# lpiccinelli-eth/UniDepth

Hardware: AMD Instinct MI355X
Metric: images/sec (whole node) + p50 latency, ViT-L/14 518x518 bs=8 (higher is better)
Workload: dtype f16; 1 GPU; UniDepthV2 vitl14 infer(), 518x518, bs=8 per GPU, all 7 outputs on device; value = 2 independent infer() calls in flight per GPU (HIP streams); value_one_call / p50_latency_ms = one call at a time; global_batch=8, parallelism=dp1, inflight=2

## Files before the change

unidepth_amd/csrc/gemm.hip:

```cpp
#include "ud_common.h"

#ifdef UD_TRACE
__device__ unsigned long long* ud_trace_ptr = nullptr;
#define UD_STAMP(slot)                                                                           \
  do {                                                                                           \
    if (ud_trace_ptr && threadIdx.x == 0 && trace_tile < 8)                                      \
      ud_trace_ptr[((size_t)blockIdx.x * 8 + trace_tile) * 8 + (slot)] = wall_clock64();         \
  } while (0)
#else
#define UD_STAMP(slot)
#endif

namespace {

constexpr int UD_LNC_TILES = 2;
constexpr int UD_LNC_PLANE = UD_LNC_TILES * 256;

template <int BN_, int WM_, int WN_>
struct Cfg {
  static constexpr int BM = 128, BN = BN_, BK = 64, WM = WM_, WN = WN_;
  static constexpr int NWM = BM / WM, NWN = BN / WN;
  static constexpr int TM = WM / 16, TN = WN / 16;
  static constexpr int A_BYTES = BM * BK * 2;
  static constexpr int B_BYTES = BN * BK * 2;
// ... 1397 lines not shown
    }
  }
  hipLaunchKernelGGL((gemm256_kernel<MH, EPI, AMODE, false, LNC, GRP>), dim3(tiles < 256 ? tiles : 256), dim3(512), lds, s, d);
  UD_CHECK_LAUNCH("ud_gemm_f16 (large tile) launch");
  return UD_OK;
}

inline int bal_cpc(const UdGemm& d) {
  const int tiles_n = (d.N + 255) >> 8;
  if (tiles_n > 128 || (d.N & 255)) return 0;
  const int cpc = 256 / tiles_n;
  const int U = (d.M + 63) >> 6;
  return (U / cpc >= 2) ? cpc : 0;
}
inline double bal_time(const UdGemm& d) {
  const int cpc = bal_cpc(d);
  if (!cpc) return 1e30;
  const int U = (d.M + 63) >> 6;
  const int un = (U + cpc - 1) / cpc;
  const int k = (un + 3) >> 2;
  return 8.0 + (un * (30.0 / 4.0) + (k - 1) * 2.5) * ((double)d.K / 1024.0);
}

template <int EPI, bool LNC = false, int AMODE = UD_A_DENSE>
int launch256bal(const UdGemm& d, hipStream_t s) {
  const int tiles_n = (d.N + 255) >> 8;
  const int cpc = bal_cpc(d);
  const int lds = 2 * BigCfg<4>::STAGE + (LNC ? LNC_LDS : 0);
  static bool attr_set[UD_MAX_DEVICES];
  if (!ud_attr_once(attr_set)) {
    if (hipFuncSetAttribute((const void*)gemm256_kernel<4, EPI, AMODE, true, LNC>, hipFuncAttributeMaxDynamicSharedMemorySize, lds) != hipSuccess) {
      ud_set_error("ud_gemm_f16: cannot reserve the LDS ring of the large-tile kernel");
      return UD_ERR_LAUNCH;
    }
  }
  hipLaunchKernelGGL((gemm256_kernel<4, EPI, AMODE, true, LNC>), dim3(cpc * tiles_n), dim3(512), lds, s, d);
  UD_CHECK_LAUNCH("ud_gemm_f16 (large tile, row-balanced) launch");
  return UD_OK;
}

inline int pick_tiles(const UdGemm& d) {
  if (d.amode == UD_A_CONV3_REFLECT || d.groups > 1 || d.M < 1024 || d.N < 192 || (d.K & 63)) return 0;
  if (d.amode == UD_A_CONV3_ZERO && d.epi != UD_EPI_F16 && d.epi != UD_EPI_F32) return 0;
  {
    const double a_bytes = d.amode == UD_A_DENSE ? 2.0 * d.M * d.lda : 2.0 * ((double)(d.M / d.rows_img) + 1.0) * (double)d.img_stride;
    if (a_bytes >= 2147483648.0 || 2.0 * d.N * d.ldw >= 2147483648.0) return 0;
  }
  if (d.epi == UD_EPI_QKV && (d.vsplit & 255)) return 0;
  if (d.tile_hint == 1 || (d.tile_hint >= 5 && d.tile_hint != 8 && d.tile_hint != 9 && d.tile_hint != 10 && (d.tile_hint < 11 || d.tile_hint > 14))) return 0;
  if (d.tile_hint >= 11 && d.tile_hint <= 14) return 3;
  if (d.tile_hint == 2) return 4;
  if (d.tile_hint == 10) return big_split_ok(d) ? 10 : 0;
  if (d.tile_hint == 3 || d.tile_hint == 9) return 3;
  const bool bal_ok = (d.amode == UD_A_DENSE || (d.amode == UD_A_CONV3_ZERO && d.epi != UD_EPI_QKV)) &&
                      (d.epi == UD_EPI_F16 || d.epi == UD_EPI_F32 || d.epi == UD_EPI_QKV) && bal_cpc(d) > 0;
  if (d.tile_hint == 8 && bal_ok) return 8;
  const double kk = (double)d.K / 1024.0;
  const double tn = (double)((d.N + 255) / 256);
  const double t256 = 8.0 + ceil(tn * ((d.M + 255) / 256) / 256.0) * 30.0 * kk;
  const double t192 = 8.0 + ceil(tn * ((d.M + 191) / 192) / 256.0) * 23.5 * kk;
  const double tbal = (bal_ok && ((d.M + 63) / 64 + bal_cpc(d) - 1) / bal_cpc(d) > 4) ? bal_time(d) : 1e30;
  const double small_tiles = (double)((d.N + 127) / 128) * ((d.M + 127) / 128);
  const double t_small = 6.0 + ceil(small_tiles / 256.0) * 0.5 * 21.5 * kk;
  double t_big = t256 <= t192 ? t256 : t192;
  int which = t256 <= t192 ? 4 : 3;
  if (tbal < 0.985 * t_big) { t_big = tbal; which = 8; }
  if (big_split_ok(d)) {
    const double tsplit = 8.0 + 0.5 * 23.5 * kk + 6.0;
    if (tsplit < t_big && tsplit < 0.93 * t_small) return 10;
  }
  if (t_big >= 0.93 * t_small) return 0;
  return which;
}

inline int big_tiles_per_wg(const UdGemm& d, int which) {
  if (which == 8) {
    const int cpc = bal_cpc(d);
    const int U = (d.M + 63) >> 6;
    return (((U + cpc - 1) / cpc) + 3) >> 2;
  }
  if (which == 10) return 1;
  const int bm = which == 3 ? 192 : 256;
  const int tiles = ((d.N + 255) >> 8) * ((d.M + bm - 1) / bm);
  return (tiles + 255) / 256;
}

template <int EPI, int AMODE = UD_A_DENSE>
int launch_big(const UdGemm& d, hipStream_t s, int which) {
  if constexpr (AMODE == UD_A_DENSE && (EPI == UD_EPI_F16 || EPI == UD_EPI_QKV)) {
    if (d.row_stats_in) {
      if (which == 8) return launch256bal<EPI, true>(d, s);
      return which == 3 ? launch256<3, EPI, AMODE, true>(d, s) : launch256<4, EPI, AMODE, true>(d, s);
    }
  }
  if constexpr (AMODE == UD_A_DENSE && (EPI == UD_EPI_F16 || EPI == UD_EPI_F32 || EPI == UD_EPI_QKV)) {
    if (which == 8 && !d.row_stats_final) return launch256bal<EPI>(d, s);
  }
  if constexpr (AMODE == UD_A_CONV3_ZERO && (EPI == UD_EPI_F16 || EPI == UD_EPI_F32)) {
    if (which == 8 && !d.row_stats_final) return launch256bal<EPI, false, UD_A_CONV3_ZERO>(d, s);
  }
  if constexpr (EPI == UD_EPI_F16 || EPI == UD_EPI_F32) {
    if (which == 10) return launch256sk<EPI, AMODE>(d, s);
  }
  if (which == 8 || which == 10) which = 3;
  return which == 3 ? launch256<3, EPI, AMODE>(d, s) : launch256<4, EPI, AMODE>(d, s);
}

constexpr int HALO_BYTES = 41 * 1024;

template <int NT, int EPI, bool REFLECT, bool UPS = false>
__global__ __launch_bounds__(256) void conv_tile_kernel(const UdGemm p) {
  extern __shared__ __attribute__((aligned(16))) char smem[];
  char* halo = smem;
  char* wbuf = smem + HALO_BYTES;
  constexpr int WB = NT * 16 * 128;
  const int tid = threadIdx.x;
  const int lane = tid & 63;
  const int wv = __builtin_amdgcn_readfirstlane(tid >> 6);
  const int tiles_x = (p.Wimg + 15) >> 4;
  const int tx = blockIdx.x % tiles_x, ty = blockIdx.x / tiles_x;
  const int x0 = tx << 4, y0 = ty << 4;
  const int b = blockIdx.y, g = blockIdx.z;
  const half_t* in = (const half_t*)p.A + (long long)g * p.gA + (long long)b * p.img_stride + p.coff;
  const half_t* W = (const half_t*)p.W + (long long)g * p.gW;
  const float* bias = p.bias + (long long)g * p.gBias;
  const float ups_sy = UPS && p.Himg > 1 ? (float)(p.Hsrc - 1) / (float)(p.Himg - 1) : 0.f;
  const float ups_sx = UPS && p.Wimg > 1 ? (float)(p.Wsrc - 1) / (float)(p.Wimg - 1) : 0.f;

  f32x4 acc[4][NT];
#pragma unroll
  for (int i = 0; i < 4; ++i)
#pragma unroll
    for (int j = 0; j < NT; ++j) acc[i][j] = (f32x4){0.f, 0.f, 0.f, 0.f};

  auto halo_coord = [&](int i, int& hp, int& cpos, int& iy, int& ix, bool& ok) {
    const int idx = i * 64 + lane;
    hp = idx >> 3;
    cpos = idx & 7;
    const int hy = hp / 18, hx = hp - hy * 18;
    iy = y0 - 1 + hy;
    ix = x0 - 1 + hx;
    ok = hp < 324;
    if constexpr (REFLECT) {
      iy = iy < 0 ? -iy : (iy >= p.Himg ? 2 * p.Himg - 2 - iy : iy);
      ix = ix < 0 ? -ix : (ix >= p.Wimg ? 2 * p.Wimg - 2 - ix : ix);
      ok = ok && iy >= 0 && ix >= 0;
    } else {
      ok = ok && (unsigned)iy < (unsigned)p.Himg && (unsigned)ix < (unsigned)p.Wimg;
    }
  };
  auto issue_halo = [&](int cc) {
    if constexpr (UPS) {
      const int ylo = y0 == 0 ? 0 : y0 - 1, yhi = y0 + 16 < p.Himg ? y0 + 16 : p.Himg - 1;
      const int xlo = x0 == 0 ? 0 : x0 - 1, xhi = x0 + 16 < p.Wimg ? x0 + 16 : p.Wimg - 1;
      const int syA = (int)(ups_sy * (float)ylo), sxA = (int)(ups_sx * (float)xlo);
      int syB = (int)(ups_sy * (float)yhi) + 1, sxB = (int)(ups_sx * (float)xhi) + 1;
      syB = syB < p.Hsrc ? syB : p.Hsrc - 1;
      sxB = sxB < p.Wsrc ? sxB : p.Wsrc - 1;
      const int PR = syB - syA + 1, PC = sxB - sxA + 1;
      char* patch = wbuf + 2 * WB;
      const int npiece = (PR * PC * 8 + 63) >> 6;
      for (int i = wv; i < npiece; i += 4) {
        const int idx = i * 64 + lane;
        int pp = idx >> 3;
        pp = pp < PR * PC ? pp : PR * PC - 1;
        const int pr = pp / PC, pc = pp - pr * PC;
        ud_glds16(in + ((long long)(syA + pr) * p.Wsrc + sxA + pc) * p.cstride + cc * 64 + ((idx & 7) << 3), patch + i * 1024);
      }
      asm volatile("s_waitcnt vmcnt(0)" ::: "memory");
      __syncthreads();
#pragma unroll
      for (int j = 0; j < 11; ++j) {
        const int i = wv + 4 * j;
        if (i < 41) {
          int hp, cpos, iy, ix;
          bool ok;
          halo_coord(i, hp, cpos, iy, ix, ok);
          ok = ok && iy >= ylo && iy <= yhi && ix >= xlo && ix <= xhi;
          half8 o8;
#pragma unroll
          for (int e = 0; e < 8; ++e) o8[e] = (half_t)0.f;
          if (ok) {
            const float fy = ups_sy * (float)iy, fx = ups_sx * (float)ix;
            const int sy0 = (int)fy, sx0 = (int)fx;
            const int sy1 = sy0 + (sy0 < p.Hsrc - 1), sx1 = sx0 + (sx0 < p.Wsrc - 1);
            const half_t ly = (half_t)(fy - (float)sy0), lx = (half_t)(fx - (float)sx0);
            const int cs = (cpos ^ ((hp >> 1) & 7)) << 4;
            const half8 h00 = *(const half8*)(patch + ((sy0 - syA) * PC + (sx0 - sxA)) * 128 + cs);
            const half8 h01 = *(const half8*)(patch + ((sy0 - syA) * PC + (sx1 - sxA)) * 128 + cs);
            const half8 h10 = *(const half8*)(patch + ((sy1 - syA) * PC + (sx0 - sxA)) * 128 + cs);
            const half8 h11 = *(const half8*)(patch + ((sy1 - syA) * PC + (sx1 - sxA)) * 128 + cs);
            const half8 top = h00 + lx * (h01 - h00);
            const half8 bot = h10 + lx * (h11 - h10);
            o8 = top + ly * (bot - top);
          }
          *(half8*)(halo + i * 1024 + lane * 16) = o8;
        }
      }
    } else {
#pragma unroll
      for (int j = 0; j < 11; ++j) {
        const int i = wv + 4 * j;
        if (i < 41) {
          int hp, cpos, iy, ix;
          bool ok;
          halo_coord(i, hp, cpos, iy, ix, ok);
          const half_t* src = ok ? in + ((long long)iy * p.Wimg + ix) * p.cstride + cc * 64 + ((cpos ^ ((hp >> 1) & 7)) << 3)
                                 : (const half_t*)p.zeros;
          ud_glds16(src, halo + i * 1024);
        }
      }
    }
  };
  auto issue_w = [&](int tap, int cc, int buf) {
#pragma unroll
    for (int j = 0; j < NT / 2; ++j) {
      const int i = wv * (NT / 2) + j;
      const int idx = i * 64 + lane;
      const int n = idx >> 3, cpos = idx & 7;
      ud_glds16(W + (size_t)n * p.ldw + tap * p.Cin + cc * 64 + ((cpos ^ ((n >> 1) & 7)) << 3), wbuf + buf * WB + i * 1024);
    }
  };

  const int px = lane & 15, fq = lane >> 4;
  const int nchunks = p.Cin >> 6;
  for (int cc = 0; cc < nchunks; ++cc) {
    __syncthreads();
    issue_halo(cc);
    issue_w(0, cc, 0);
#pragma unroll 1
    for (int tap = 0; tap < 9; ++tap) {
      asm volatile("s_waitcnt vmcnt(0)" ::: "memory");
      __syncthreads();
      if (tap < 8) issue_w(tap + 1, cc, (tap + 1) & 1);
      const int t3 = (tap * 11) >> 5;
      const int dy = t3, dx = tap - t3 * 3;
      const char* wb = wbuf + (tap & 1) * WB;
#pragma unroll
      for (int ks = 0; ks < 2; ++ks) {
        half8 af[4], bf[NT];
#pragma unroll
        for (int i = 0; i < 4; ++i) {
          const int hp = (wv * 4 + i + dy) * 18 + px + dx;
          af[i] = *(const half8*)(halo + hp * 128 + (((ks * 4 + fq) ^ ((hp >> 1) & 7)) << 4));
        }
#pragma unroll
        for (int j = 0; j < NT; ++j) {
          const int n = j * 16 + px;
          bf[j] = *(const half8*)(wb + n * 128 + (((ks * 4 + fq) ^ ((n >> 1) & 7)) << 4));
        }
#pragma unroll
        for (int i = 0; i < 4; ++i)
#pragma unroll
          for (int j = 0; j < NT; ++j) acc[i][j] = __builtin_amdgcn_mfma_f32_16x16x32_f16(bf[j], af[i], acc[i][j], 0, 0, 0);
      }
    }
  }

#pragma unroll
  for (int i = 0; i < 4; ++i) {
    const int y = y0 + wv * 4 + i, x = x0 + px;
    const bool ok = y < p.Himg && x < p.Wimg;
    const size_t row = ((size_t)b * p.Himg + y) * p.Wimg + x;
    if constexpr (EPI == UD_EPI_HEAD) {
      const float* w2 = p.w2 + (long long)g * p.gW2;
      float part = 0.f;
#pragma unroll
      for (int j = 0; j < NT; ++j) {
        const int nb = j * 16 + 4 * fq;
        const f32x4 bv = *(const f32x4*)(bias + nb);
        const f32x4 wv2 = *(const f32x4*)(w2 + nb);
#pragma unroll
        for (int r = 0; r < 4; ++r) part += ud_lrelu(acc[i][j][r] + bv[r]) * wv2[r];
      }
      part += __shfl_xor(part, 16, 64);
      part += __shfl_xor(part, 32, 64);
      if (ok && fq == 0) {
        float yv = part + (g == 0 ? p.b2 : p.b2_g1);
        yv = fminf(fmaxf(yv, -8.0f), 8.0f);
        ((float*)p.out)[(long long)g * p.gOut + row] = __expf(yv + (g == 0 ? p.post_add : p.post_add_g1));
      }
    } else {
      if (ok) {
        const bool lre = p.act == UD_ACT_LRELU;
        half_t* o = (half_t*)p.out + (long long)g * p.gOut + row * p.ldc;
#pragma unroll
        for (int j = 0; j < NT; ++j) {
          const int nb = j * 16 + 4 * fq;
          const f32x4 bv = *(const f32x4*)(bias + nb);
          half4 h;
#pragma unroll
          for (int r = 0; r < 4; ++r) {
            const float t = acc[i][j][r] + bv[r];
            h[r] = (half_t)(lre ? ud_lrelu(t) : t);
          }
          *(half4*)(o + nb) = h;
        }
      }
    }
  }
}


__global__ __launch_bounds__(256, 2) void conv_head_regw_kernel(const UdGemm p, const int tiles_x, const int tiles_img, const int tiles_g) {
  extern __shared__ __attribute__((aligned(16))) char smem[];
  char* halo = smem;
  char* patch = smem + HALO_BYTES;
  const int tid = threadIdx.x;
  const int lane = tid & 63;
  const int wv = __builtin_amdgcn_readfirstlane(tid >> 6);
  const int g = blockIdx.y;
  const int px = lane & 15, fq = lane >> 4;
  const half_t* W = (const half_t*)p.W + (long long)g * p.gW;
  const float* bias = p.bias + (long long)g * p.gBias;
  const float* w2 = p.w2 + (long long)g * p.gW2;
  const float ups_sy = p.Himg > 1 ? (float)(p.Hsrc - 1) / (float)(p.Himg - 1) : 0.f;
  const float ups_sx = p.Wimg > 1 ? (float)(p.Wsrc - 1) / (float)(p.Wimg - 1) : 0.f;

  half8 bfr[9][2][2];
#pragma unroll
  for (int tap = 0; tap < 9; ++tap)
#pragma unroll
    for (int ks = 0; ks < 2; ++ks)
#pragma unroll
      for (int j = 0; j < 2; ++j) bfr[tap][ks][j] = *(const half8*)(W + (size_t)(j * 16 + px) * p.ldw + tap * 64 + (ks * 4 + fq) * 8);
  struct Geo { int b, x0, y0, ylo, yhi, xlo, xhi, syA, sxA, PR, PC; };
  auto geo = [&](int t) {
    Geo q;
    q.b = __builtin_amdgcn_readfirstlane(t / tiles_img);
    const int r = t - q.b * tiles_img;
    const int ty = __builtin_amdgcn_readfirstlane(r / tiles_x), tx = r - ty * tiles_x;
    q.x0 = tx << 4; q.y0 = ty << 4;
    q.ylo = q.y0 == 0 ? 0 : q.y0 - 1; q.yhi = q.y0 + 16 < p.Himg ? q.y0 + 16 : p.Himg - 1;
    q.xlo = q.x0 == 0 ? 0 : q.x0 - 1; q.xhi = q.x0 + 16 < p.Wimg ? q.x0 + 16 : p.Wimg - 1;
    q.syA = (int)(ups_sy * (float)q.ylo); q.sxA = (int)(ups_sx * (float)q.xlo);
    int syB = (int)(ups_sy * (float)q.yhi) + 1, sxB = (int)(ups_sx * (float)q.xhi) + 1;
    syB = syB < p.Hsrc ? syB : p.Hsrc - 1;
    sxB = sxB < p.Wsrc ? sxB : p.Wsrc - 1;
    q.syA = __builtin_amdgcn_readfirstlane(q.syA); q.sxA = __builtin_amdgcn_readfirstlane(q.sxA);
    q.PR = __builtin_amdgcn_readfirstlane(syB - q.syA + 1); q.PC = __builtin_amdgcn_readfirstlane(sxB - q.sxA + 1);
    return q;
  };
  auto issue_patch = [&](const Geo& q) {
    const half_t* in = (const half_t*)p.A + (long long)g * p.gA + (long long)q.b * p.img_stride + p.coff;
    const int npiece = (q.PR * q.PC * 8 + 63) >> 6;
    for (int i = wv; i < npiece; i += 4) {
      const int idx = i * 64 + lane;
      int pp = idx >> 3;
      pp = pp < q.PR * q.PC ? pp : q.PR * q.PC - 1;
      const int pr = pp / q.PC, pc = pp - pr * q.PC;
      ud_glds16(in + ((long long)(q.syA + pr) * p.Wsrc + q.sxA + pc) * p.cstride + ((idx & 7) << 3), patch + i * 1024);
    }
  };

  int t = __builtin_amdgcn_readfirstlane(blockIdx.x);
  if (t >= tiles_g) return;
  Geo cur = geo(t);
  issue_patch(cur);
  for (; t < tiles_g; t += gridDim.x) {
    asm volatile("s_waitcnt vmcnt(0)" ::: "memory");
    __syncthreads();
#pragma unroll 1
    for (int jj = 0; jj < 11; ++jj) {
      const int i = wv + 4 * jj;
      if (i < 41) {
        const int idx = i * 64 + lane;
        const int hp = idx >> 3, cpos = idx & 7;
        const int hy = hp / 18, hx = hp - hy * 18;
        int iy = cur.y0 - 1 + hy, ix = cur.x0 - 1 + hx;
        iy = iy < 0 ? -iy : (iy >= p.Himg ? 2 * p.Himg - 2 - iy : iy);
        ix = ix < 0 ? -ix : (ix >= p.Wimg ? 2 * p.Wimg - 2 - ix : ix);
        const bool ok = hp < 324 && iy >= cur.ylo && iy <= cur.yhi && ix >= cur.xlo && ix <= cur.xhi;
        half8 o8;
#pragma unroll
        for (int e = 0; e < 8; ++e) o8[e] = (half_t)0.f;
        if (ok) {
          const float fy = ups_sy * (float)iy, fx = ups_sx * (float)ix;
          const int sy0 = (int)fy, sx0 = (int)fx;
          const int sy1 = sy0 + (sy0 < p.Hsrc - 1), sx1 = sx0 + (sx0 < p.Wsrc - 1);
          const half_t ly = (half_t)(fy - (float)sy0), lx = (half_t)(fx - (float)sx0);
          const int cs = (cpos ^ ((hp >> 1) & 7)) << 4;
          const half8 h00 = *(const half8*)(patch + ((sy0 - cur.syA) * cur.PC + (sx0 - cur.sxA)) * 128 + cs);
          const half8 h01 = *(const half8*)(patch + ((sy0 - cur.syA) * cur.PC + (sx1 - cur.sxA)) * 128 + cs);
          const half8 h10 = *(const half8*)(patch + ((sy1 - cur.syA) * cur.PC + (sx0 - cur.sxA)) * 128 + cs);
          const half8 h11 = *(const half8*)(patch + ((sy1 - cur.syA) * cur.PC + (sx1 - cur.sxA)) * 128 + cs);
          const half8 top = h00 + lx * (h01 - h00);
          const half8 bot = h10 + lx * (h11 - h10);
          o8 = top + ly * (bot - top);
        }
        *(half8*)(halo + i * 1024 + lane * 16) = o8;
      }
    }
    __syncthreads();
    const int tn = t + (int)gridDim.x;
    Geo nxt = cur;
    if (tn < tiles_g) {
      nxt = geo(tn);
      issue_patch(nxt);
    }
    f32x4 acc[4][2];
#pragma unroll
    for (int i = 0; i < 4; ++i)
#pragma unroll
      for (int j = 0; j < 2; ++j) acc[i][j] = (f32x4){0.f, 0.f, 0.f, 0.f};
#pragma unroll
    for (int tap = 0; tap < 9; ++tap) {
      const int dy = tap / 3, dx = tap - dy * 3;
#pragma unroll
      for (int ks = 0; ks < 2; ++ks) {
        half8 af[4];
#pragma unroll
        for (int i = 0; i < 4; ++i) {
          const int hp = (wv * 4 + i + dy) * 18 + px + dx;
          af[i] = *(const half8*)(halo + hp * 128 + (((ks * 4 + fq) ^ ((hp >> 1) & 7)) << 4));
        }
#pragma unroll
        for (int i = 0; i < 4; ++i)
#pragma unroll
          for (int j = 0; j < 2; ++j) acc[i][j] = __builtin_amdgcn_mfma_f32_16x16x32_f16(bfr[tap][ks][j], af[i], acc[i][j], 0, 0, 0);
        __builtin_amdgcn_sched_barrier(0);
      }
    }
    f32x4 bv[2], wv2[2];
#pragma unroll
    for (int j = 0; j < 2; ++j) {
      bv[j] = *(const f32x4*)(bias + j * 16 + 4 * fq);
      wv2[j] = *(const f32x4*)(w2 + j * 16 + 4 * fq);
    }
#pragma unroll
    for (int i = 0; i < 4; ++i) {
      const int y = cur.y0 + wv * 4 + i, x = cur.x0 + px;
      const bool ok = y < p.Himg && x < p.Wimg;
      const size_t row = ((size_t)cur.b * p.Himg + y) * p.Wimg + x;
      float part = 0.f;
#pragma unroll
      for (int j = 0; j < 2; ++j)
#pragma unroll
        for (int r = 0; r < 4; ++r) part += ud_lrelu(acc[i][j][r] + bv[j][r]) * wv2[j][r];
      part += __shfl_xor(part, 16, 64);
      part += __shfl_xor(part, 32, 64);
      if (ok && fq == 0) {
        float yv = part + (g == 0 ? p.b2 : p.b2_g1);
        yv = fminf(fmaxf(yv, -8.0f), 8.0f);
        ((float*)p.out)[(long long)g * p.gOut + row] = __expf(yv + (g == 0 ? p.post_add : p.post_add_g1));
      }
    }
    cur = nxt;
  }
}

constexpr int UPS_PATCH = 13;
template <int NT, int EPI, bool REFLECT, bool UPS = false>
int launch_conv_tile(const UdGemm& d, hipStream_t s) {
  const int lds = HALO_BYTES + 2 * NT * 16 * 128 + (UPS ? (UPS_PATCH * UPS_PATCH * 128 + 1023) / 1024 * 1024 : 0);
  if (UPS) {
    static bool attr_set[UD_MAX_DEVICES];
    if (!ud_attr_once(attr_set)) (void)hipFuncSetAttribute((const void*)conv_tile_kernel<NT, EPI, REFLECT, UPS>, hipFuncAttributeMaxDynamicSharedMemorySize, lds);
  }
  const int B = d.M / d.rows_img;
  dim3 grid(((d.Wimg + 15) >> 4) * ((d.Himg + 15) >> 4), B, d.groups > 0 ? d.groups : 1);
  hipLaunchKernelGGL((conv_tile_kernel<NT, EPI, REFLECT, UPS>), grid, dim3(256), lds, s, d);
  UD_CHECK_LAUNCH("ud_gemm_f16 (halo-tile conv) launch");
  return UD_OK;
}

inline bool head_regw_enabled() { return true; }

inline bool conv_tile_ok(const UdGemm& d) {
  return d.amode != UD_A_DENSE && d.a_wrap == 0 && (d.N == 32 || d.N == 64) && (d.Cin & 63) == 0 && d.rows_img == d.Himg * d.Wimg &&
         d.M % d.rows_img == 0 && d.bias != nullptr && d.tile_hint != 1 && d.Himg >= 2 && d.Wimg >= 2 &&
         (d.epi == UD_EPI_HEAD || (d.epi == UD_EPI_F16 && d.act != UD_ACT_GELU && d.rows_in == 0 && d.add == nullptr && (d.ldc & 3) == 0));
}

inline int ring_variant(const UdGemm& d) {
  const int tiles = ((d.N + 127) / 128) * ((d.M + 127) / 128);
  const int nkt = d.K >> 6;
  if (d.amode != UD_A_DENSE || d.N <= 64 || (d.epi != UD_EPI_F16 && d.epi != UD_EPI_F32 && d.epi != UD_EPI_QKV)) return 0;
  if (!(d.groups <= 1 && nkt >= 4 && d.tile_hint != 5 && ((tiles <= 256 && nkt >= 8) || d.tile_hint >= 6) && !(ud_debug_flags_host() & 16))) return 0;
  if (d.epi != UD_EPI_QKV && d.splitk_ws && d.splitk_cnt && tiles <= 128 && (nkt & 1) == 0 && (nkt >= 16 || (d.tile_hint == 7 && nkt >= 8)) &&
      d.tile_hint != 6 && !(ud_debug_flags_host() & 32))
    return 2;
  return 1;
}

template <class C, int EPI, int AMODE>
int launch(const UdGemm& d, hipStream_t s) {
  const int tiles_n = (d.N + C::BN - 1) / C::BN;
  const int tiles_m = (d.M + C::BM - 1) / C::BM;
  if constexpr (C::BN == 128 && AMODE == UD_A_DENSE && (EPI == UD_EPI_F16 || EPI == UD_EPI_F32 || EPI == UD_EPI_QKV)) {
    const int variant = ring_variant(d);
    if (variant) {
      const int lds4 = 4 * C::STAGE_BYTES;
      if constexpr (EPI == UD_EPI_F16 || EPI == UD_EPI_F32) {
        if (variant == 2) {
          static bool attrs_set[UD_MAX_DEVICES];
          if (!ud_attr_once(attrs_set)) {
            if (hipFuncSetAttribute((const void*)gemm_kernel<C, EPI, AMODE, 4, true>, hipFuncAttributeMaxDynamicSharedMemorySize, lds4) != hipSuccess) {
              ud_set_error("ud_gemm_f16: cannot reserve the 4-stage LDS ring");
              return UD_ERR_LAUNCH;
            }
          }
          hipLaunchKernelGGL((gemm_kernel<C, EPI, AMODE, 4, true>), dim3(2 * tiles_m * tiles_n), dim3(256), lds4, s, d);
          UD_CHECK_LAUNCH("ud_gemm_f16 (4-stage ring, K split) launch");
          return UD_OK;
        }
      }
      static bool attr4_set[UD_MAX_DEVICES];
      if (!ud_attr_once(attr4_set)) {
        if (hipFuncSetAttribute((const void*)gemm_kernel<C, EPI, AMODE, 4>, hipFuncAttributeMaxDynamicSharedMemorySize, lds4) != hipSuccess) {
          ud_set_error("ud_gemm_f16: cannot reserve the 4-stage LDS ring");
          return UD_ERR_LAUNCH;
        }
      }
      hipLaunchKernelGGL((gemm_kernel<C, EPI, AMODE, 4>), dim3(tiles_m * tiles_n), dim3(256), lds4, s, d);
      UD_CHECK_LAUNCH("ud_gemm_f16 (4-stage ring) launch");
      return UD_OK;
    }
  }
  const int lds = 2 * C::STAGE_BYTES;
  static bool attr_set[UD_MAX_DEVICES];
  if (!ud_attr_once(attr_set)) (void)hipFuncSetAttribute((const void*)gemm_kernel<C, EPI, AMODE>, hipFuncAttributeMaxDynamicSharedMemorySize, lds);
  dim3 grid(tiles_m * tiles_n, 1, d.groups > 0 ? d.groups : 1);
  hipLaunchKernelGGL((gemm_kernel<C, EPI, AMODE>), grid, dim3(256), lds, s, d);
  UD_CHECK_LAUNCH("ud_gemm_f16 launch");
  return UD_OK;
}

template <int EPI, int AMODE>
int dispatch_bn(const UdGemm& d, hipStream_t s) {
  if (d.N > 64) return launch<Cfg<128, 64, 64>, EPI, AMODE>(d, s);
  if (d.N > 32) return launch<Cfg<64, 64, 32>, EPI, AMODE>(d, s);
  return launch<Cfg<32, 32, 32>, EPI, AMODE>(d, s);
}

inline bool grouped_as_big(const UdGemm& d, UdGemm& m) {
  if (d.groups <= 1 || d.amode != UD_A_DENSE || (d.M & 255) || d.tile_hint == 1 || d.a_wrap || d.w_wrap || d.row_stats_in || d.row_stats_out || d.max_out ||
      d.rows_in || d.add)
    return false;
#ifdef UD_AB_PREV
  if (d.epi != UD_EPI_F16 && d.epi != UD_EPI_QKV) return false;
#endif
  if (d.epi != UD_EPI_F16 && d.epi != UD_EPI_QKV && !(d.epi == UD_EPI_F32 && (d.tile_hint == 2 || (d.accumulate == 0 && d.K >= 1024)))) return false;
  if (!(d.gA == 0 || d.gA == (long long)d.M * d.lda) || d.gOut != (long long)d.M * d.ldc) return false;
  if (d.bias && d.gBias < 0) return false;
  if (d.out2) {
    if (d.epi == UD_EPI_QKV) {
      if (d.tok_per_img <= 0 || d.M % d.tok_per_img || d.gOut2 != (long long)(d.M / d.tok_per_img) * d.heads_v * 64 * d.kv_ld) return false;
    } else if (d.gOut2 != (long long)d.M * d.ldc2) {
      return false;
    }
  }
  m = d;
  m.grp_rows = d.M;
  m.M = d.M * d.groups;
  m.groups = 1;
  if (2.0 * (double)d.groups * d.N * d.ldw >= 2147483648.0 || 2.0 * (double)m.M * d.lda >= 2147483648.0) return false;
  m.tile_hint = 0;
  const int bt = pick_tiles(m);
  return bt == 4 || bt == 3 || bt == 8;
}

}

bool ud_gemm_pp_ok(const UdGemm& d);
int ud_gemm_pp_launch(const UdGemm& d, hipStream_t s);
bool ud_gemm_duo_ok(const UdGemm& d);
int ud_gemm_duo_launch(const UdGemm& d, hipStream_t s, int prio_mode);
namespace {
inline bool pp_pick(const UdGemm& d) {
#ifdef UD_AB_PREV
  return false;
#endif
  if (!ud_gemm_pp_ok(d)) return false;
  if (d.tile_hint == 11) return true;
  if (d.tile_hint != 0) return false;
  const int tiles = (d.N >> 8) * ((d.M + 191) / 192);
  return tiles <= 256 && tiles >= 128 && pick_tiles(d) == 3;
}
}

extern "C" int ud_gemm_f16(const UdGemm* desc, void* stream) {
  UdGemm dcopy = *desc;
  if ((ud_debug_flags_host() & 4) && (dcopy.epi == UD_EPI_F16 || dcopy.epi == UD_EPI_QKV)) dcopy.ldc2 |= (1 << 30);
  if (ud_debug_flags_host() & 8) dcopy.tile_hint = 1;
  const UdGemm& d = dcopy;
  hipStream_t s = (hipStream_t)stream;
  if (!d.A || !d.W || !d.out || d.M <= 0 || d.N <= 0 || d.K <= 0 || (d.K & 63) || (d.N & 3)) {
    ud_set_error("ud_gemm_f16: bad argument (need K % 64 == 0, N % 4 == 0)");
    return UD_ERR_BAD_ARG;
  }
  if (d.a_wrap < 0 || d.w_wrap < 0 || (d.amode == UD_A_DENSE ? (d.a_wrap & 63) : (d.a_wrap & 7)) || (d.w_wrap & 63) ||
      (d.a_wrap && d.w_wrap) || (d.w_wrap && d.amode != UD_A_DENSE) || (d.a_wrap && d.amode == UD_A_DENSE && 2 * d.a_wrap < d.K) ||
      (d.w_wrap && 2 * d.w_wrap < d.K) || (d.a_wrap && d.amode != UD_A_DENSE && 2 * d.a_wrap < d.Cin) ||
      ((d.a_wrap || d.w_wrap) && (d.amode == UD_A_CONV3_REFLECT_UP || d.groups > 1 && d.amode != UD_A_DENSE))) {
    ud_set_error("ud_gemm_f16: bad a_wrap / w_wrap (one operand may wrap, once: 2 * wrap >= K resp. Cin; dense: multiple of 64, conv: of 8)");
    return UD_ERR_BAD_ARG;
  }
  if (d.row_stats_in) {
    const int bt = d.amode == UD_A_DENSE ? pick_tiles(d) : 0;
    if (d.amode != UD_A_DENSE || (d.epi != UD_EPI_F16 && d.epi != UD_EPI_QKV) || !d.wsum || d.add || d.rows_in || (d.N & 15) || bt == 0) {
      ud_set_error("ud_gemm_f16: LayerNorm-folded consumer (row_stats_in) needs dense A, an fp16 epilogue without add / row remap, wsum, N % 16 == 0 "
                   "and a problem the large-tile kernel takes (ud_gemm_pick >= 3)");
      return UD_ERR_UNSUPPORTED;
    }
  }
  if (d.max_out && (d.epi != UD_EPI_F32 || d.rows_in || d.accumulate == 2)) {
    ud_set_error("ud_gemm_f16: max_out needs the fp32 epilogue without a row remap");
    return UD_ERR_UNSUPPORTED;
  }
  if (d.row_stats_out) {
    const int bt = d.amode == UD_A_DENSE || d.amode == UD_A_CONV3_ZERO ? pick_tiles(d) : 0;
    if (d.epi != UD_EPI_F32 || (d.N & 63) || (bt == 0 && (d.N <= 64 || d.groups > 1))) {
      ud_set_error("ud_gemm_f16: row_stats_out needs the fp32 epilogue, N % 64 == 0 and 64-column wave tiles (N > 64, no groups)");
      return UD_ERR_UNSUPPORTED;
    }
    if (d.row_stats_final && (bt == 0 || !d.row_stats_ticket || d.ln_D <= 0 || d.N > 1024 || (d.N & 127) || d.groups > 1)) {
      ud_set_error("ud_gemm_f16: row_stats_final (in-kernel reduction of the row statistics) needs the large-tile kernel, a ticket buffer, ln_D, "
                   "N <= 1024 and N % 128 == 0 (the finalizer reads the 64-column slabs in pairs)");
      return UD_ERR_UNSUPPORTED;
    }
  } else if (d.row_stats_final) {
    ud_set_error("ud_gemm_f16: row_stats_final without row_stats_out");
    return UD_ERR_BAD_ARG;
  }
  if (d.amode == UD_A_CONV3_REFLECT_UP && d.epi != UD_EPI_HEAD) {
    ud_set_error("ud_gemm_f16: CONV3_REFLECT_UP is implemented for the HEAD epilogue only");
    return UD_ERR_UNSUPPORTED;
  }
  if (d.amode != UD_A_DENSE && (!d.zeros || (d.Cin & 7) || d.K < 9 * d.Cin || d.rows_img < d.Himg * d.Wimg)) {
    ud_set_error("ud_gemm_f16: bad conv geometry");
    return UD_ERR_BAD_ARG;
  }
  if (d.epi == UD_EPI_QKV) {
    if (d.amode != UD_A_DENSE || !d.out2 || (d.vsplit % 128) || (d.tok_per_img & 3) || (d.kv_ld & 3) || d.N <= 64) {
      ud_set_error("ud_gemm_f16: bad QKV epilogue geometry");
      return UD_ERR_BAD_ARG;
    }
    {
      UdGemm mg;
      if (grouped_as_big(d, mg)) return launch256<4, UD_EPI_QKV, UD_A_DENSE, false, true>(mg, s);
    }
    if (const int bt = pick_tiles(d)) return launch_big<UD_EPI_QKV>(d, s, bt);
    return launch<Cfg<128, 64, 64>, UD_EPI_QKV, UD_A_DENSE>(d, s);
  }
  if (d.up_src && d.epi != UD_EPI_D2S) {
    ud_set_error("ud_gemm_f16: up_src belongs to the D2S epilogue");
    return UD_ERR_BAD_ARG;
  }
  if (d.epi == UD_EPI_D2S) {
    if (d.amode != UD_A_DENSE || (d.d2s_Co & 3)) {
      ud_set_error("ud_gemm_f16: bad D2S epilogue geometry");
      return UD_ERR_BAD_ARG;
    }
    if (d.up_src && (d.up_H < 1 || d.up_W < 1 || 2 * d.up_H != d.d2s_Hin * d.d2s_k || 2 * d.up_W != d.d2s_Win * d.d2s_k || (d.up_ld & 3) || d.up_ld < d.d2s_Co ||
                     d.up_img_rows < d.up_H * d.up_W || d.groups > 1)) {
      ud_set_error("ud_gemm_f16: up_src (fused x2 up-sampling under the D2S accumulate) needs 2 * up_H == d2s_Hin * d2s_k (same for W), up_ld % 4 == 0, "
                   "up_ld >= d2s_Co, up_img_rows >= up_H * up_W");
      return UD_ERR_BAD_ARG;
    }
    if (const int bt = pick_tiles(d)) return launch_big<UD_EPI_D2S>(d, s, bt);
    return dispatch_bn<UD_EPI_D2S, UD_A_DENSE>(d, s);
  }
  if (d.epi == UD_EPI_HEAD) {
    if ((d.amode != UD_A_CONV3_REFLECT && d.amode != UD_A_CONV3_REFLECT_UP) || d.N != 32 || !d.w2 || !d.bias) {
      ud_set_error("ud_gemm_f16: HEAD epilogue needs reflect conv, N == 32");
      return UD_ERR_BAD_ARG;
    }
    if (d.amode == UD_A_CONV3_REFLECT_UP) {
      const bool fits = 17.0 * (d.Hsrc - 1) / (d.Himg > 1 ? d.Himg - 1 : 1) + 3.0 <= UPS_PATCH && 17.0 * (d.Wsrc - 1) / (d.Wimg > 1 ? d.Wimg - 1 : 1) + 3.0 <= UPS_PATCH;
      if (!conv_tile_ok(d) || d.Hsrc < 1 || d.Wsrc < 1 || (d.cstride & 7) || !fits) {
        ud_set_error("ud_gemm_f16: CONV3_REFLECT_UP needs Cin % 64 == 0, dense images, Hsrc / Wsrc >= 1 and an up-sampling factor >= ~1.7");
        return UD_ERR_BAD_ARG;
      }
      if (d.Cin == 64 && head_regw_enabled()) {
        const int lds = HALO_BYTES + (UPS_PATCH * UPS_PATCH * 128 + 1023) / 1024 * 1024;
        static bool attr_set[UD_MAX_DEVICES];
        if (!ud_attr_once(attr_set)) (void)hipFuncSetAttribute((const void*)conv_head_regw_kernel, hipFuncAttributeMaxDynamicSharedMemorySize, lds);
        const int B = d.M / d.rows_img;
        const int tiles_x = (d.Wimg + 15) >> 4, tiles_img = tiles_x * ((d.Himg + 15) >> 4), tiles_g = tiles_img * B;
        const int G = d.groups > 0 ? d.groups : 1;
        int wgs = (512 + G - 1) / G;
        wgs = wgs < tiles_g ? wgs : tiles_g;
        hipLaunchKernelGGL(conv_head_regw_kernel, dim3(wgs, G), dim3(256), lds, s, d, tiles_x, tiles_img, tiles_g);
        UD_CHECK_LAUNCH("ud_gemm_f16 (head conv, register-resident weights) launch");
        return UD_OK;
      }
      return launch_conv_tile<2, UD_EPI_HEAD, true, true>(d, s);
    }
    if (conv_tile_ok(d)) return launch_conv_tile<2, UD_EPI_HEAD, true>(d, s);
    return launch<Cfg<32, 32, 32>, UD_EPI_HEAD, UD_A_CONV3_REFLECT>(d, s);
  }
  if (d.epi == UD_EPI_F16) {
    if (conv_tile_ok(d)) {
      if (d.amode == UD_A_CONV3_REFLECT) return d.N == 64 ? launch_conv_tile<4, UD_EPI_F16, true>(d, s) : launch_conv_tile<2, UD_EPI_F16, true>(d, s);
      return d.N == 64 ? launch_conv_tile<4, UD_EPI_F16, false>(d, s) : launch_conv_tile<2, UD_EPI_F16, false>(d, s);
    }
    {
      UdGemm mg;
      if (grouped_as_big(d, mg)) return launch256<4, UD_EPI_F16, UD_A_DENSE, false, true>(mg, s);
    }
    if (const int bt = pick_tiles(d))
      return d.amode == UD_A_DENSE ? launch_big<UD_EPI_F16>(d, s, bt) : launch_big<UD_EPI_F16, UD_A_CONV3_ZERO>(d, s, bt);
    if (d.amode == UD_A_DENSE) return dispatch_bn<UD_EPI_F16, UD_A_DENSE>(d, s);
    if (d.amode == UD_A_CONV3_ZERO) return dispatch_bn<UD_EPI_F16, UD_A_CONV3_ZERO>(d, s);
    return dispatch_bn<UD_EPI_F16, UD_A_CONV3_REFLECT>(d, s);
  }
  if (d.epi == UD_EPI_F32) {
    {
      UdGemm mg;
      if (grouped_as_big(d, mg)) return launch256<4, UD_EPI_F32, UD_A_DENSE, false, true>(mg, s);
    }
    if (d.tile_hint >= 12 && d.tile_hint <= 14 && ud_gemm_duo_ok(d)) return ud_gemm_duo_launch(d, s, d.tile_hint == 12 ? 1 : d.tile_hint == 13 ? 0 : 2);
    if (pp_pick(d)) return ud_gemm_pp_launch(d, s);
    if (const int bt = pick_tiles(d))
      return d.amode == UD_A_DENSE ? launch_big<UD_EPI_F32>(d, s, bt) : launch_big<UD_EPI_F32, UD_A_CONV3_ZERO>(d, s, bt);
    if (d.amode == UD_A_DENSE) return dispatch_bn<UD_EPI_F32, UD_A_DENSE>(d, s);
    if (d.amode == UD_A_CONV3_ZERO) return dispatch_bn<UD_EPI_F32, UD_A_CONV3_ZERO>(d, s);
  }
  ud_set_error("ud_gemm_f16: unsupported epi/amode combination");
  return UD_ERR_UNSUPPORTED;
}

#ifdef UD_TRACE
extern "C" int ud_trace_set(void* buf) {
// ... 25 lines not shown
```

Baseline: 632.6 images/s.

## Restructure conv head halo upsampling with row tables and reuse halo loads across taps

The halo build in the fused upsample+3x3 conv head kernel is reorganized so each lane handles a fixed x column and channel chunk across several rows. Per-row source coordinates and weights are precomputed once per lane and shared with ds_bpermute, and packed f16 FMA lerps replace the scalar ones. The MFMA loop now walks halo rows, loading each halo fragment once and reusing it for every output row/tap that needs it, with double-buffered prefetch of the next fragment. This cuts LDS reads and index arithmetic, but the swizzle pattern for halo writes changes and must match the reader's XOR layout. There is also some added register pressure.

```diff
diff --git a/unidepth_amd/csrc/gemm.hip b/unidepth_amd/csrc/gemm.hip
--- a/unidepth_amd/csrc/gemm.hip
+++ b/unidepth_amd/csrc/gemm.hip
@@ -1723,6 +1723,30 @@
 }
 
 
+__device__ __forceinline__ void ud_ups_coord(const float scale, const int i, int& i0, half_t& w) {
+  float f = scale * (float)i;
+  asm("" : "+v"(f));
+  i0 = (int)f;
+  w = (half_t)(f - (float)i0);
+}
+
+__device__ __forceinline__ half2v ud_pk_sub_f16(const half2v b, const half2v a) {
+  half2v d;
+  asm("v_pk_add_f16 %0, %1, %2 neg_lo:[0,1] neg_hi:[0,1]" : "=v"(d) : "v"(b), "v"(a));
+  return d;
+}
+__device__ __forceinline__ half8 ud_lerp8(const half8& a, const half8& b, const half2v w) {
+  half8 r;
+#pragma unroll
+  for (int e = 0; e < 4; ++e) {
+    const half2v a2 = {a[2 * e], a[2 * e + 1]}, b2 = {b[2 * e], b[2 * e + 1]};
+    const half2v o = __builtin_elementwise_fma(w, ud_pk_sub_f16(b2, a2), a2);
+    r[2 * e] = o[0];
+    r[2 * e + 1] = o[1];
+  }
+  return r;
+}
+
 __global__ __launch_bounds__(256, 2) void conv_head_regw_kernel(const UdGemm p, const int tiles_x, const int tiles_img, const int tiles_g) {
   extern __shared__ __attribute__((aligned(16))) char smem[];
   char* halo = smem;
@@ -1765,8 +1789,10 @@
   auto issue_patch = [&](const Geo& q) {
     const half_t* in = (const half_t*)p.A + (long long)g * p.gA + (long long)q.b * p.img_stride + p.coff;
     const int npiece = (q.PR * q.PC * 8 + 63) >> 6;
+    int lp = lane;
+    asm volatile("" : "+v"(lp));
     for (int i = wv; i < npiece; i += 4) {
-      const int idx = i * 64 + lane;
+      const int idx = i * 64 + lp;
       int pp = idx >> 3;
       pp = pp < q.PR * q.PC ? pp : q.PR * q.PC - 1;
       const int pr = pp / q.PC, pc = pp - pr * q.PC;
@@ -1781,35 +1807,54 @@
   for (; t < tiles_g; t += gridDim.x) {
     asm volatile("s_waitcnt vmcnt(0)" ::: "memory");
     __syncthreads();
-#pragma unroll 1
-    for (int jj = 0; jj < 11; ++jj) {
-      const int i = wv + 4 * jj;
-      if (i < 41) {
-        const int idx = i * 64 + lane;
-        const int hp = idx >> 3, cpos = idx & 7;
-        const int hy = hp / 18, hx = hp - hy * 18;
-        int iy = cur.y0 - 1 + hy, ix = cur.x0 - 1 + hx;
-        iy = iy < 0 ? -iy : (iy >= p.Himg ? 2 * p.Himg - 2 - iy : iy);
-        ix = ix < 0 ? -ix : (ix >= p.Wimg ? 2 * p.Wimg - 2 - ix : ix);
-        const bool ok = hp < 324 && iy >= cur.ylo && iy <= cur.yhi && ix >= cur.xlo && ix <= cur.xhi;
-        half8 o8;
-#pragma unroll
-        for (int e = 0; e < 8; ++e) o8[e] = (half_t)0.f;
-        if (ok) {
-          const float fy = ups_sy * (float)iy, fx = ups_sx * (float)ix;
-          const int sy0 = (int)fy, sx0 = (int)fx;
-          const int sy1 = sy0 + (sy0 < p.Hsrc - 1), sx1 = sx0 + (sx0 < p.Wsrc - 1);
-          const half_t ly = (half_t)(fy - (float)sy0), lx = (half_t)(fx - (float)sx0);
-          const int cs = (cpos ^ ((hp >> 1) & 7)) << 4;
-          const half8 h00 = *(const half8*)(patch + ((sy0 - cur.syA) * cur.PC + (sx0 - cur.sxA)) * 128 + cs);
-          const half8 h01 = *(const half8*)(patch + ((sy0 - cur.syA) * cur.PC + (sx1 - cur.sxA)) * 128 + cs);
-          const half8 h10 = *(const half8*)(patch + ((sy1 - cur.syA) * cur.PC + (sx0 - cur.sxA)) * 128 + cs);
-          const half8 h11 = *(const half8*)(patch + ((sy1 - cur.syA) * cur.PC + (sx1 - cur.sxA)) * 128 + cs);
-          const half8 top = h00 + lx * (h01 - h00);
-          const half8 bot = h10 + lx * (h11 - h10);
-          o8 = top + ly * (bot - top);
-        }
-        *(half8*)(halo + i * 1024 + lane * 16) = o8;
+    int ln = lane;
+    asm volatile("" : "+v"(ln));
+    int rowtab;
+    {
+      const int iy = cur.y0 - 1 + (ln < 18 ? ln : 17);
+      const int iyr = iy < 0 ? -iy : (iy >= p.Himg ? 2 * p.Himg - 2 - iy : iy);
+      const bool ok = iyr >= cur.ylo && iyr <= cur.yhi;
+      int sy0;
+      half_t ly;
+      ud_ups_coord(ups_sy, ok ? iyr : cur.ylo, sy0, ly);
+      rowtab = (int)ok | ((sy0 < p.Hsrc - 1) << 1) | ((sy0 - cur.syA) * cur.PC * 128) | ((int)__builtin_bit_cast(unsigned short, ly) << 16);
+    }
+    const int task = wv * 64 + ln;
+    if (task < 216) {
+      const int seg = task >= 144 ? 2 : (task >= 72 ? 1 : 0);
+      const int rem = task - seg * 72;
+      const int hx = rem >> 2, cp = rem & 3;
+      const int ix = cur.x0 - 1 + hx;
+      const int ixr = ix < 0 ? -ix : (ix >= p.Wimg ? 2 * p.Wimg - 2 - ix : ix);
+      const bool okx = ixr >= cur.xlo && ixr <= cur.xhi;
+      int sx0;
+      half_t lx;
+      ud_ups_coord(ups_sx, okx ? ixr : cur.xlo, sx0, lx);
+      const half2v lx2 = {lx, lx};
+      const char* q0 = patch + (sx0 - cur.sxA) * 128 + cp * 16;
+      const char* q1 = q0 + (sx0 < p.Wsrc - 1 ? 128 : 0);
+      const int rowstep = cur.PC * 128;
+#pragma unroll 2
+      for (int r = 0; r < 6; ++r) {
+        const int hy = seg * 6 + r;
+        const int e = __builtin_amdgcn_ds_bpermute(hy << 2, rowtab);
+        const int ra = e & 0xff80, rb = ra + ((e & 2) ? rowstep : 0);
+        const half_t ly = __builtin_bit_cast(half_t, (unsigned short)((unsigned)e >> 16));
+        const half2v ly2 = {ly, ly};
+        const bool ok = okx && (e & 1);
+        const int hp = hy * 18 + hx;
+        const int slot = hp * 128 + ((cp ^ ((hp >> 1) & 3)) << 4) + (((hp >> 3) & 1) << 6);
+#pragma unroll
+        for (int k = 0; k < 2; ++k) {
+          const half8 h00 = *(const half8*)(q0 + ra + k * 64), h01 = *(const half8*)(q1 + ra + k * 64);
+          const half8 h10 = *(const half8*)(q0 + rb + k * 64), h11 = *(const half8*)(q1 + rb + k * 64);
+          half8 o = ud_lerp8(ud_lerp8(h00, h01, lx2), ud_lerp8(h10, h11, lx2), ly2);
+          if (!ok) {
+#pragma unroll
+            for (int j = 0; j < 8; ++j) o[j] = (half_t)0.f;
+          }
+          *(half8*)(halo + (slot ^ (k << 6))) = o;
+        }
       }
     }
     __syncthreads();
@@ -1824,23 +1869,29 @@
     for (int i = 0; i < 4; ++i)
 #pragma unroll
       for (int j = 0; j < 2; ++j) acc[i][j] = (f32x4){0.f, 0.f, 0.f, 0.f};
-#pragma unroll
-    for (int tap = 0; tap < 9; ++tap) {
-      const int dy = tap / 3, dx = tap - dy * 3;
-#pragma unroll
-      for (int ks = 0; ks < 2; ++ks) {
-        half8 af[4];
-#pragma unroll
-        for (int i = 0; i < 4; ++i) {
-          const int hp = (wv * 4 + i + dy) * 18 + px + dx;
-          af[i] = *(const half8*)(halo + hp * 128 + (((ks * 4 + fq) ^ ((hp >> 1) & 7)) << 4));
-        }
-#pragma unroll
-        for (int i = 0; i < 4; ++i)
-#pragma unroll
-          for (int j = 0; j < 2; ++j) acc[i][j] = __builtin_amdgcn_mfma_f32_16x16x32_f16(bfr[tap][ks][j], af[i], acc[i][j], 0, 0, 0);
-        __builtin_amdgcn_sched_barrier(0);
-      }
+    half8 af[2][2];
+    auto load_unit = [&](int u, half8* f) {
+      const int hp = (wv * 4 + u / 3) * 18 + px + u % 3;
+#pragma unroll
+      for (int ks = 0; ks < 2; ++ks) f[ks] = *(const half8*)(halo + hp * 128 + (((ks * 4 + fq) ^ ((hp >> 1) & 7)) << 4));
+    };
+    load_unit(0, af[0]);
+#pragma unroll
+    for (int u = 0; u < 18; ++u) {
+      const int h = u / 3, dx = u % 3;
+      if (u + 1 < 18) load_unit(u + 1, af[(u + 1) & 1]);
+#pragma unroll
+      for (int i = 0; i < 4; ++i) {
+        const int dy = h - i;
+        if (dy >= 0 && dy <= 2) {
+#pragma unroll
+          for (int ks = 0; ks < 2; ++ks)
+#pragma unroll
+            for (int j = 0; j < 2; ++j)
+              acc[i][j] = __builtin_amdgcn_mfma_f32_16x16x32_f16(bfr[dy * 3 + dx][ks][j], af[u & 1][ks], acc[i][j], 0, 0, 0);
+        }
+      }
+      __builtin_amdgcn_sched_barrier(0);
     }
     f32x4 bv[2], wv2[2];
 #pragma unroll
```

New measurement: 637.7 images/s, median of 6. No clear change (+0.8%).
